# EDM-Research/Real-time-Neural-Rendering-of-LiDAR-Point-Clouds

Measured on AMD Instinct MI355X. Metric: Mpoints/sec projected + frames/sec at 1920x1080, higher is better.
Workload: dtype f32

## Files before the change

real-time-neural-rendering-of-lidar-point-clouds_amd/csrc/rtr_kernels.h:

```cpp
#pragma once
#include <hip/hip_runtime.h>
#include <stdint.h>

#include "rtr_chunk_box.h"

namespace rtr {

struct Proj {
    float m[12];
};

constexpr uint32_t kPackMaxBits = 25;
struct PackedXyz {
    const uint4 *hdr;
    const uint32_t *planes;
    const uint32_t *planes_b;
};
constexpr uint64_t pack_b_dwords(uint64_t units) { return (units * 2 + 256 + 16 + 15) & ~15ull; }
constexpr uint64_t pack_total_dwords(uint64_t units) { return pack_b_dwords(units) + units * 6 + 16; }

struct Cloud {
    const float *x, *y, *z;
    const uint32_t *rgba;
    uint64_t n;
    int grid;
    int incoherent;
    PackedXyz pk;
    const float *spread;
    float absmax[3];
    Clip clip;
    Keep keep;
};

struct FilterLevels {
    float *lv[9];
    int w[9], h[9];
    int levels;
};

constexpr int kMaxPeers = 16;
struct PeerSet {
    void *p[kMaxPeers];
};
struct OwnedTab;
struct Sliced {
    PeerSet src;
    size_t chunk;
    const uint32_t *occ_all;
    int peers;
    uint32_t *out;
    int rank;
    const OwnedTab *tab;
};
struct OwnedTab {
    const uint32_t *meta[kMaxPeers];
    const uint64_t *ext0[kMaxPeers];
    const uint64_t *dyn[kMaxPeers];
    const uint32_t *depth[kMaxPeers];
    const uint8_t *ximg[kMaxPeers];
};
struct TilePyr {
    FilterLevels L;
    uint32_t n_eff_rows;
    uint32_t *part_min, *part_max;
    int enable;
};
constexpr int kS0Shift = 12;
constexpr uint32_t kS0 = 1u << kS0Shift;
constexpr int kDirK = 21;
constexpr int kHeavyExtra = 512;
struct TileStore {
    uint64_t *ext0;
    uint32_t *meta;
    uint32_t seq;
    int nst, ntiles;
    int fill_shift;
};
constexpr int kFillShiftMax = 6;
struct StoreConsts {
    uint32_t *depth, *acc, *occ;
    uint64_t *dyn;
    uint64_t dyn_cap;
    uint32_t heavy, slice;
    uint32_t *err_host;
    uint32_t *split_host;
    uint32_t *entries_host;
};
__host__ __device__ constexpr size_t ts_align4(size_t x) { return (x + 3) & ~(size_t)3; }
__host__ __device__ constexpr size_t ts_off_count(int nst, int nt) { return ts_align4((size_t)nst << kFillShiftMax); }
__host__ __device__ constexpr size_t ts_off_tile_cnt(int nst, int nt) { return ts_off_count(nst, nt) + ts_align4((size_t)nst); }
__host__ __device__ constexpr size_t ts_off_hctr(int nst, int nt) { return ts_off_tile_cnt(nst, nt) + ts_align4((size_t)nt); }
__host__ __device__ constexpr size_t ts_off_items(int nst, int nt) { return ts_off_hctr(nst, nt) + ts_align4((size_t)nt); }
__host__ __device__ constexpr size_t ts_off_hdr(int nst, int nt) { return ts_off_items(nst, nt) + ((size_t)2 * nt + kHeavyExtra + 1) * 8; }
__host__ __device__ constexpr size_t ts_off_ticket(int nst, int nt) { return ts_off_hdr(nst, nt) + 32; }
__host__ __device__ constexpr size_t ts_off_pool(int nst, int nt) { return ts_off_ticket(nst, nt) + 2; }
__host__ __device__ constexpr size_t ts_off_dir(int nst, int nt) { return ts_off_pool(nst, nt) + 2; }
__host__ __device__ constexpr size_t ts_off_perm(int nst, int nt) { return ts_off_dir(nst, nt) + (size_t)nst * kDirK * 2; }
__host__ __device__ constexpr size_t ts_off_dbg(int nst, int nt) { return ts_off_perm(nst, nt) + ts_align4((size_t)nt); }
__host__ __device__ constexpr size_t ts_off_cnt4(int nst, int nt) { return ts_align4(ts_off_dbg(nst, nt) + 128); }
constexpr int kSubTickets = 32;
__host__ __device__ constexpr size_t ts_off_sub(int nst, int nt) { return ts_off_cnt4(nst, nt) + (size_t)nt * 4; }
__host__ __device__ constexpr size_t ts_off_order(int nst, int nt) { return ts_off_sub(nst, nt) + (size_t)kSubTickets * 32; }
// ... 204 lines not shown
```

real-time-neural-rendering-of-lidar-point-clouds_amd/csrc/rtr_kernels.hip:

```cpp
#include "rtr_device.h"
#include "rtr_lane_test.h"
#include "rtr_remove_index.h"
#include "rtr_extract_index.h"

#include <hip/hip_ext.h>
#include <hip/hip_fp16.h>

#include <type_traits>

namespace rtr {

__global__ __launch_bounds__(kBlock) void k_clear(uint4 *__restrict__ depth4, uint4 *__restrict__ acc4,
                                                  size_t n_depth4, size_t n_acc4, uint32_t *depth, size_t npix) {
    size_t i = (size_t)blockIdx.x * kBlock + threadIdx.x;
    size_t stride = (size_t)gridDim.x * kBlock;
    const uint4 e = make_uint4(RTR_EMPTY, RTR_EMPTY, RTR_EMPTY, RTR_EMPTY);
    const uint4 z = make_uint4(0, 0, 0, 0);
    for (size_t j = i; j < n_acc4; j += stride) acc4[j] = z;
    for (size_t j = i; j < n_depth4; j += stride) depth4[j] = e;
    for (size_t j = n_depth4 * 4 + i; j < npix; j += stride) depth[j] = RTR_EMPTY;
}

void launch_clear(hipStream_t s, uint32_t *depth, uint32_t *acc, size_t npix) {
    size_t n_acc4 = npix, n_depth4 = npix / 4;
// ... 263 lines not shown
                 project_point(P, X1.z, Y1.z, Z1.z, W, H, fW, fH, d) ^ project_point(P, X1.w, Y1.w, Z1.w, W, H, fW, fH, d);
        }
        if (i < n4) {
            Quad q = project_quad(x4, y4, z4, i, P, W, H, fW, fH);
            h += (uint32_t)(q.pix[0] ^ q.pix[1] ^ q.pix[2] ^ q.pix[3]);
        }
    } else {
        for (uint64_t i = (uint64_t)blockIdx.x * kBlock + threadIdx.x; i < n4; i += stride) {
            if (V == 0) {
                Quad q = project_quad(x4, y4, z4, i, P, W, H, fW, fH);
                h += (uint32_t)(q.pix[0] ^ q.pix[1] ^ q.pix[2] ^ q.pix[3]);
            } else if (V == 3) {
                float4 X = x4[i], Y = y4[i], Z = z4[i];
                float d;
                h += project_point(P, X.x, Y.x, Z.x, W, H, fW, fH, d) ^ project_point(P, X.y, Y.y, Z.y, W, H, fW, fH, d) ^
                     project_point(P, X.z, Y.z, Z.z, W, H, fW, fH, d) ^ project_point(P, X.w, Y.w, Z.w, W, H, fW, fH, d);
            } else if (V == 4) {
                float4 X = ld_stream(x4 + i), Y = ld_stream(y4 + i), Z = ld_stream(z4 + i);
                h += __float_as_uint(X.x) ^ __float_as_uint(Y.y) ^ __float_as_uint(Z.z) ^ __float_as_uint(X.w) ^
                     __float_as_uint(Y.x) ^ __float_as_uint(Z.y);
            } else {
                float4 X = ld_stream(x4 + i), Y = ld_stream(y4 + i), Z = ld_stream(z4 + i);
                const float xs[4] = {X.x, X.y, X.z, X.w}, ys[4] = {Y.x, Y.y, Y.z, Y.w}, zs[4] = {Z.x, Z.y, Z.z, Z.w};
#pragma unroll
                for (int k = 0; k < 4; ++k) {
                    float rx = f_add(fmaf(P.m[2], zs[k], fmaf(P.m[1], ys[k], f_mul(P.m[0], xs[k]))), P.m[3]);
                    float ry = f_add(fmaf(P.m[6], zs[k], fmaf(P.m[5], ys[k], f_mul(P.m[4], xs[k]))), P.m[7]);
                    float rz = f_add(fmaf(P.m[10], zs[k], fmaf(P.m[9], ys[k], f_mul(P.m[8], xs[k]))), P.m[11]);
                    float inv = __builtin_amdgcn_rcpf(rz);
                    float fu = rintf(f_mul(rx, inv)), fv = rintf(f_mul(ry, inv));
                    bool ok = (rz > 0.0f) && (fu >= 0.0f) && (fu < fW) && (fv >= 0.0f) && (fv < fH);
                    h += ok ? (uint32_t)((int)fv * W + (int)fu) : 0xFFFFFFFFu;
                }
            }
        }
    }
    if (h == 0x12345678u) sink[0] = h;
}

void launch_stream_probe(hipStream_t s, const Cloud &c, const Proj &P, int W, int H, uint32_t *sink, int variant) {
    uint64_t n4 = (c.n + 3) / 4;
    if (n4 == 0) return;
    dim3 g(point_grid(n4, c.grid)), b(kBlock);
    const float4 *x = (const float4 *)c.x, *y = (const float4 *)c.y, *z = (const float4 *)c.z;
    switch (variant) {
        case 1: hipLaunchKernelGGL(k_stream_probe<1>, g, b, 0, s, x, y, z, n4, P, W, H, sink); break;
        case 2: hipLaunchKernelGGL(k_stream_probe<2>, g, b, 0, s, x, y, z, n4, P, W, H, sink); break;
        case 3: hipLaunchKernelGGL(k_stream_probe<3>, g, b, 0, s, x, y, z, n4, P, W, H, sink); break;
        case 4: hipLaunchKernelGGL(k_stream_probe<4>, g, b, 0, s, x, y, z, n4, P, W, H, sink); break;
        default: hipLaunchKernelGGL(k_stream_probe<0>, g, b, 0, s, x, y, z, n4, P, W, H, sink); break;
    }
}

constexpr int kTileH = 32;
#ifndef RTR_TILE_THREADS
#define RTR_TILE_THREADS 512
#define RTR_TILE_BATCH 8
#define RTR_TILE_WAVES 6
#endif
constexpr int kTileThreads = RTR_TILE_THREADS;
#ifndef RTR_TILE0_THREADS
#define RTR_TILE0_THREADS 256
#endif
constexpr int kTileThreadsCompact = RTR_TILE0_THREADS;
#ifndef RTR_TILE0_WAVES
#define RTR_TILE0_WAVES 8
#define RTR_TILE0_SWEEP 4
#endif
#ifndef RTR_TILE0_HEAD
#define RTR_TILE0_HEAD 1
#endif
#ifndef RTR_TILE0_AHEAD
#define RTR_TILE0_AHEAD 1
#endif
#ifndef RTR_TILE0_BATCH
#define RTR_TILE0_BATCH 8
#endif
constexpr int kTileBatch = RTR_TILE_BATCH;
#ifndef RTR_T1_RING
#define RTR_T1_RING 3
#endif
#ifndef RTR_T1_LEAD
#define RTR_T1_LEAD 4
#endif
#ifndef RTR_T1_WAVES
#define RTR_T1_WAVES 5
#endif
constexpr int kSplitGrid = 256;
constexpr int kPer2 = kTileBatch / 2, kPer4 = kTileBatch / 4;
constexpr int kMaxGroups = RTR_MAX_GROUPS;
constexpr int kMaxSegs = 4 * kDirK;
#ifdef RTR_EXPERIMENT
#define RTR_XP(bit) ((xp & (bit)) != 0)
#define RTR_STAMP(S, slot) do { if (threadIdx.x == 0) ts_dbg(S)[slot] = wall_clock64(); } while (0)
#else
#define RTR_XP(bit) false
#define RTR_STAMP(S, slot) do { } while (0)
#endif

struct TileGeom {
    int tw_shift;
    int tiles_x, tiles_y, ntiles;
    int stx, sty, nst;
};

__host__ __device__ inline TileGeom tile_geom(int W, int H) {
    TileGeom g;
    g.tw_shift = 5;
    g.tiles_x = (W + 31) >> 5;
    g.tiles_y = (H + kTileH - 1) / kTileH;
    if (g.tiles_x * g.tiles_y > 4096) {
        g.tw_shift = 6;
        g.tiles_x = (W + 63) >> 6;
    }
    g.ntiles = g.tiles_x * g.tiles_y;
    g.stx = (W + 31) >> 5;
    g.sty = (H + 15) >> 4;
    g.nst = g.stx * g.sty;
    return g;
}

int tile_count(int W, int H) { return tile_geom(W, H).ntiles; }
int storage_tile_count(int W, int H) { return tile_geom(W, H).nst; }

__device__ __forceinline__ unsigned long long make_entry(uint32_t depth_bits, uint32_t pix9, uint32_t colour) {
    return ((unsigned long long)depth_bits << 33) | ((unsigned long long)pix9 << 24) | (unsigned long long)(colour & 0xFFFFFFu);
}

__device__ __forceinline__ void store_error(const TileStore &S, uint32_t code) { atomicOr(ts_hdr(S) + kHdrErrLive, code); }
__device__ __forceinline__ void store_error_now(const TileStore &S, uint32_t code) {
    store_error(S, code);
    typedef uint32_t __attribute__((address_space(1))) *gu32_t;
    uint32_t *const host = ts_consts(S)->err_host;
    if (host) *(volatile gu32_t)host = code;
}

__device__ __forceinline__ unsigned long long extent_alloc(const TileStore &S, uint32_t st, uint32_t v) {
    const int k = 32 - __clz((int)(v >> kS0Shift));
    const uint32_t start = kS0 << (k - 1);
    if (v != start) return 0ull;
    const unsigned long long base = atomicAdd(ts_pool(S), (unsigned long long)start);
    const unsigned long long e = (base << 24) | (unsigned long long)S.seq;
    __hip_atomic_store(ts_dir(S) + (size_t)st * kDirK + k, e, __ATOMIC_RELAXED, __HIP_MEMORY_SCOPE_AGENT);
    return e;
}
__device__ __forceinline__ uint64_t *extent_slot(const TileStore &S, uint32_t st, uint32_t v, unsigned long long own) {
    const int k = 32 - __clz((int)(v >> kS0Shift));
    const uint32_t start = kS0 << (k - 1);
    unsigned long long e = own;
    if (e == 0ull) {
        const unsigned long long *d = ts_dir(S) + (size_t)st * kDirK + k;
        int polls = 0;
        for (;;) {
            e = __hip_atomic_load(d, __ATOMIC_RELAXED, __HIP_MEMORY_SCOPE_AGENT);
            if ((uint32_t)(e & 0xFFFFFFull) == S.seq) break;
            if (++polls > (1 << 22)) {
                store_error(S, 1u);
                return nullptr;
            }
            __builtin_amdgcn_s_sleep(4);
        }
    }
    const unsigned long long base = e >> 24;
    const StoreConsts *sc = ts_consts(S);
    if (base + start > sc->dyn_cap) {
        store_error(S, 2u);
// ... 266 lines not shown
    if (threadIdx.x == 0) {
        sum = mx = over = 0;
        for (int k = 0; k < nw; ++k) {
            sum += s_w[k];
            mx = s_w[8 + k] > mx ? s_w[8 + k] : mx;
            over += s_w[16 + k];
        }
        uint32_t *const hdr = ts_hdr(S);
        hdr[kHdrItems] = (uint32_t)S.ntiles;
        hdr[kHdrSplitItems] = 0u;
        hdr[kHdrEntries] = sum;
        hdr[kHdrHeaviest] = mx;
        hdr[kHdrSlice] = sc->slice < 1u ? 1u : sc->slice;
        hdr[kHdrSplitTiles] = 0u;
        typedef uint32_t __attribute__((address_space(1))) *gu32_t;
        if (sc->split_host) *(volatile gu32_t)sc->split_host = over ? 1u : 0u;
        if (sc->entries_host) *(volatile gu32_t)sc->entries_host = sum;
        *flag = 0u;
    }
}
__device__ void lean_frame_end(const TileStore &S, int parity) {
    uint32_t *const hdr = ts_hdr(S);
    const int t = threadIdx.x;
    if (t < 64) {
        unsigned long long cc = 0ull;
        if (t < kSubTickets) {
            cc = *ts_sub_colour(S, (uint32_t)t);
            *ts_sub_colour(S, (uint32_t)t) = 0ull;
        }
        uint32_t c32 = (uint32_t)cc;
#pragma unroll
        for (int off = 32; off > 0; off >>= 1) c32 += __shfl_xor(c32, off, 64);
        if (t == 0) {
            hdr[kHdrColourChunks] = c32;
            const StoreConsts *const sc = ts_consts(S);
            const uint32_t err = __hip_atomic_load(hdr + kHdrErrLive, __ATOMIC_RELAXED, __HIP_MEMORY_SCOPE_AGENT);
            hdr[kHdrError] = err;
            if (err) {
                typedef uint32_t __attribute__((address_space(1))) *gu32_t;
                hdr[kHdrErrLive] = 0u;
                if (sc->err_host) *(volatile gu32_t)sc->err_host = err;
            }
            *ts_pool(S) = 0ull;
            ts_lflag(S)[parity] = 1u;
        }
    }
    __shared__ uint32_t s_fold[24];
    lean_fold(S, parity ^ 1, s_fold);
    __syncthreads();
    next_frame_order(S, parity, true);
}
__global__ __launch_bounds__(kBlock) void k_lean_fold(TileStore S, int parity) {
    __shared__ uint32_t s_fold[24];
    lean_fold(S, parity, s_fold);
}
void launch_lean_fold(hipStream_t s, int W, int H, const TileStore &S, int parity) {
    (void)W, (void)H;
    hipLaunchKernelGGL(k_lean_fold, dim3(1), dim3(kBlock), 0, s, S, parity);
}


struct ViewTab {
    Proj P[kMaxViews];
    LaneTest lt[kMaxViews];
    TileStore S[kMaxViews];
    const float *spread;
    int count;
};

template <bool CULL, bool GROUPS, bool PACKED, bool CTEST, bool MV, class... Filter>
__global__ __launch_bounds__(kBlock, (PACKED && !CULL && !MV) ? RTR_T1_WAVES : 4) void k_project_bin(const float4 *__restrict__ x4, const float4 *__restrict__ y4,
                                                        const float4 *__restrict__ z4,
                                                        const uint4 *__restrict__ rgba4, uint32_t n4, Proj P, int W,
                                                        int H, TileStore S, const float *__restrict__ bounds,
                                                        int clear_split, uint32_t cblock, int xp, LaneTest lt, Filter... filter) {
    constexpr bool CLIP = sizeof...(Filter) > 0, KEEP = sizeof...(Filter) > 1;
    const Clip no_clip{};
    const Keep no_keep{};
    const Clip &clip = filter_clip(no_clip, filter...);
    const Keep &kmask = filter_keep(no_keep, filter...);
    (void)xp;
    const ViewTab *const vt = MV ? reinterpret_cast<const ViewTab *>(bounds) : nullptr;
    const float *const spread = CULL ? nullptr : (MV ? vt->spread : bounds);
    const bool lane_test = (clear_split & 4) == 0;
    const uint4 *const pk_hdr = reinterpret_cast<const uint4 *>(x4);
    const uint32_t *const pk_planes = reinterpret_cast<const uint32_t *>(y4);
    const uint32_t *const pk_planes_b = reinterpret_cast<const uint32_t *>(z4);
    const float fW = (float)W, fH = (float)H;
    const float hiW = f_add(fW, 0.25f), hiH = f_add(fH, 0.25f);
    const int lane = threadIdx.x & 63;
    const uint32_t stx = (uint32_t)(W + 31) >> 5;
    uint32_t *fill = ts_fill(S);
    const uint32_t nchunks = (n4 + 63u) / 64u, NW = gridDim.x * (kBlock / 64), wave = blockIdx.x * (kBlock / 64) + (threadIdx.x >> 6);
    const uint32_t R = (nchunks + NW - 1u) / NW;
#ifdef RTR_EXPERIMENT
    const unsigned long long t_wave0 = wall_clock64();
    if (lane == 0 && (wave & 63u) == 0u) atomicMax(ts_dbg(S) + 59, ~t_wave0);
#endif
    const uint32_t auto_groups = ts_hdr(S)[kHdrEntries] > n4 ? 16u : ((PACKED && !CULL && GROUPS && R >= 16u) ? 5u : 1u);
    const uint32_t G = cblock < 1u ? auto_groups : (cblock > gridDim.x ? gridDim.x : cblock);
    const uint32_t phase = (uint32_t)((uint64_t)((blockIdx.x * G) / gridDim.x) * R / G);
    auto chunk_of = [&](uint32_t q) -> uint32_t {
        uint32_t r = q + phase;
        r = r >= R ? r - R : r;
        const uint32_t c = r * NW + wave;
        return (q < R && c < nchunks) ? c : nchunks;
    };
    struct Rows { float4 X, Y, Z; float rz[4]; };
    float mv[12];
#pragma unroll
    for (int k = 0; k < 12; ++k) {
        mv[k] = P.m[k];
        asm volatile("" : "+v"(mv[k]));
    }
    float nzfront = -lt.zfront;
    if constexpr (!PACKED) asm volatile("" : "+v"(nzfront));
    auto use_view = [&](uint32_t v) {
        if constexpr (MV) {
            S = vt->S[v];
            fill = ts_fill(S);
#pragma unroll
            for (int k = 0; k < 12; ++k) {
                mv[k] = vt->P[v].m[k];
                asm volatile("" : "+v"(mv[k]));
            }
            lt = vt->lt[v];
            nzfront = -lt.zfront;
            if constexpr (!PACKED) asm volatile("" : "+v"(nzfront));
        } else {
            (void)v;
        }
    };
#define RTR_M(k) mv[k]
    auto project_rows = [&](const float4 &X, const float4 &Y, const float4 &Z, Rows &r) {
        const float xs[4] = {X.x, X.y, X.z, X.w}, ys[4] = {Y.x, Y.y, Y.z, Y.w}, zs[4] = {Z.x, Z.y, Z.z, Z.w};
        r.X = X, r.Y = Y, r.Z = Z;
#pragma unroll
        for (int k = 0; k < 4; ++k) r.rz[k] = f_add(fmaf(RTR_M(10), zs[k], fmaf(RTR_M(9), ys[k], f_mul(RTR_M(8), xs[k]))), RTR_M(11));
    };
    auto lane_maybe = [&](float x0, float y0, float z0, float sp, bool live) -> bool {
        const float rz0 = f_add(fmaf(RTR_M(10), z0, fmaf(RTR_M(9), y0, f_mul(RTR_M(8), x0))), RTR_M(11));
        const float sz = f_mul(sp, lt.lz);
        const bool front = live && (f_add(rz0, sz) > nzfront);
        if (__ballot(front) == 0ull) return false;
        const float rx0 = f_add(fmaf(RTR_M(2), z0, fmaf(RTR_M(1), y0, f_mul(RTR_M(0), x0))), RTR_M(3));
        const float ry0 = f_add(fmaf(RTR_M(6), z0, fmaf(RTR_M(5), y0, f_mul(RTR_M(4), x0))), RTR_M(7));
        const float m = fminf(fminf(fmaf(hiW, rz0, -rx0), fmaf(hiH, rz0, -ry0)), fminf(fmaf(0.75f, rz0, rx0), fmaf(0.75f, rz0, ry0)));
        const bool out = (int)(f_sub(rz0, sz) > lt.zsafe) & (int)(m < -f_mul(sp, lt.lall));
        return __ballot(front && !out) != 0ull;
    };
    uint32_t n_colour = 0;
    uint32_t kst = kKeepAll;
    (void)kst;
    auto do_quad = [&](uint32_t i, bool live, const Rows &r) {
        const float *rz = r.rz;
        const bool front = live && (fmaxf(fmaxf(rz[0], rz[1]), fmaxf(rz[2], rz[3])) > 0.0f);
        if (__ballot(front) == 0ull) return;
        float rx[4], ry[4];
        {
            const float xs[4] = {r.X.x, r.X.y, r.X.z, r.X.w}, ys[4] = {r.Y.x, r.Y.y, r.Y.z, r.Y.w}, zs[4] = {r.Z.x, r.Z.y, r.Z.z, r.Z.w};
#pragma unroll
            for (int k = 0; k < 4; ++k) {
                rx[k] = f_add(fmaf(RTR_M(2), zs[k], fmaf(RTR_M(1), ys[k], f_mul(RTR_M(0), xs[k]))), RTR_M(3));
                ry[k] = f_add(fmaf(RTR_M(6), zs[k], fmaf(RTR_M(5), ys[k], f_mul(RTR_M(4), xs[k]))), RTR_M(7));
            }
        }
        bool maybe[4], any = false;
#pragma unroll
        for (int k = 0; k < 4; ++k) {
            const float z = rz[k];
            const float m = fminf(fminf(fmaf(hiW, z, -rx[k]), fmaf(hiH, z, -ry[k])), fminf(fmaf(0.75f, z, rx[k]), fmaf(0.75f, z, ry[k])));
            const bool out = (z > 1e-30f) && (m < 0.0f);
            maybe[k] = live && (z > 0.0f) && !out;
            any = any || maybe[k];
        }
        if (__ballot(any) == 0ull || RTR_XP(64)) return;
        if constexpr (CLIP) {
            const float xs[4] = {r.X.x, r.X.y, r.X.z, r.X.w}, ys[4] = {r.Y.x, r.Y.y, r.Y.z, r.Y.w}, zs[4] = {r.Z.x, r.Z.y, r.Z.z, r.Z.w};
            any = false;
#pragma unroll
            for (int k = 0; k < 4; ++k) {
                maybe[k] = maybe[k] && clip_keep(clip, xs[k], ys[k], zs[k]);
                any = any || maybe[k];
            }
            if (__ballot(any) == 0ull) return;
        }
        if constexpr (KEEP) {
            if (kst != kKeepAll) {
                const uint32_t c = (uint32_t)__builtin_amdgcn_readfirstlane((int)(i >> 6));
                const uint32_t kb = keep_bits(kmask, c, (uint32_t)lane);
                any = false;
#pragma unroll
                for (int k = 0; k < 4; ++k) {
                    maybe[k] = maybe[k] && ((kb >> k) & 1u);
                    any = any || maybe[k];
                }
                if (__ballot(any) == 0ull) return;
            }
        }
        bool in[4];
        uint32_t st[4], pix[4];
        unsigned long long pm[4];
#pragma unroll
        for (int k = 0; k < 4; ++k) {
            in[k] = false;
            st[k] = 0;
            pix[k] = 0;
            pm[k] = 0ull;
            if (__ballot(maybe[k]) == 0ull) continue;
            float inv = 1.0f / rz[k];
            float fu = rintf(f_mul(rx[k], inv));
            float fv = rintf(f_mul(ry[k], inv));
            in[k] = maybe[k] && (fu >= 0.0f) && (fu < fW) && (fv >= 0.0f) && (fv < fH);
            pm[k] = __ballot(in[k]);
            if (in[k]) {
                const int u = (int)fu, v = (int)fv;
                st[k] = (uint32_t)(v >> 4) * stx + (uint32_t)(u >> 5);
                pix[k] = (uint32_t)(((v & 15) << 5) | (u & 31));
            }
        }
        if ((pm[0] | pm[1] | pm[2] | pm[3]) == 0ull || RTR_XP(8)) return;
        n_colour += 1u;
        const uint4 col = rgba4[i];
        int grp[4] = {-1, -1, -1, -1};
        uint32_t rank[4] = {0, 0, 0, 0};
        uint32_t covered = 0;
#pragma clang diagnostic push
#pragma clang diagnostic ignored "-Wuninitialized"
#pragma clang diagnostic ignored "-Wsometimes-uninitialized"
        uint32_t claim[kMaxGroups];
#pragma clang diagnostic pop
        int ng = 0;
#pragma unroll
        for (int it = 0; it < (GROUPS ? kMaxGroups : 0); ++it) {
            const int kk = pm[0] ? 0 : (pm[1] ? 1 : (pm[2] ? 2 : (pm[3] ? 3 : -1)));
            if (kk < 0) continue;
            const unsigned long long pk = kk == 0 ? pm[0] : (kk == 1 ? pm[1] : (kk == 2 ? pm[2] : pm[3]));
            const uint32_t sk = kk == 0 ? st[0] : (kk == 1 ? st[1] : (kk == 2 ? st[2] : st[3]));
            const int first = __ffsll((long long)pk) - 1;
            const uint32_t lead = (uint32_t)__builtin_amdgcn_readlane((int)sk, first);
            uint32_t total = 0, lower = 0;
            bool gk[4];
#pragma unroll
            for (int k = 0; k < 4; ++k) {
                const unsigned long long m = __ballot(st[k] == lead) & pm[k];
                gk[k] = __builtin_amdgcn_inverse_ballot_w64(m);
                lower += __builtin_amdgcn_mbcnt_hi((uint32_t)(m >> 32), __builtin_amdgcn_mbcnt_lo((uint32_t)m, 0u));
                total += (uint32_t)__popcll(m);
                pm[k] &= ~m;
            }
#pragma unroll
            for (int k = 0; k < 4; ++k)
                if (gk[k]) {
                    grp[k] = it;
                    rank[k] = lower++;
                }
            if (lane == it) claim[it] = atomicAdd(fill + ((size_t)lead << S.fill_shift), total);
            ng = it + 1;
            covered += total;
            if (it == 3 && covered <= 8u) {
                pm[0] = pm[1] = pm[2] = pm[3] = 0ull;
            }
        }
#pragma unroll
        for (int k = 0; k < 4; ++k)
            if (in[k] && grp[k] < 0) {
                rank[k] = atomicAdd(fill + ((size_t)st[k] << S.fill_shift), 1u);
                grp[k] = kMaxGroups;
            }
        uint32_t bsel[4] = {0u, 0u, 0u, 0u};
        auto select_base = [&](auto self, auto it_tag) -> void {
            constexpr int it = decltype(it_tag)::value;
            if constexpr (it < kMaxGroups) {
                if (it < ng) {
                    const uint32_t b_it = (uint32_t)__builtin_amdgcn_readlane((int)claim[it], it);
#pragma unroll
                    for (int k = 0; k < 4; ++k) bsel[k] = grp[k] == it ? b_it : bsel[k];
                    self(self, std::integral_constant<int, it + 1>{});
                }
            }
        };
        if (!RTR_XP(16)) select_base(select_base, std::integral_constant<int, 0>{});
        const uint32_t cs[4] = {col.x, col.y, col.z, col.w};
        uint32_t v[4];
        bool dyn = false;
#pragma unroll
        for (int k = 0; k < 4; ++k) {
            v[k] = bsel[k] + rank[k];
            dyn = dyn || (in[k] && v[k] >= kS0);
        }
        if (RTR_XP(4)) return;
        if (RTR_XP(512)) {
            if ((v[0] ^ v[1] ^ v[2] ^ v[3]) == 0x7FFFFFFFu) fill[0] = 0u;
            return;
        }
        if (__ballot(dyn) == 0ull) {
            const bool quad = in[0] && in[1] && in[2] && in[3] && grp[0] < kMaxGroups && grp[0] == grp[1] &&
                              grp[0] == grp[2] && grp[0] == grp[3];
            if (quad) {
                typedef unsigned long long ull2 __attribute__((ext_vector_type(2)));
                struct __attribute__((packed, aligned(8))) Pair { ull2 v; };
                Pair *dst = reinterpret_cast<Pair *>(S.ext0 + ((size_t)st[0] << kS0Shift) + v[0]);
                ull2 a, b;
                a.x = make_entry(__float_as_uint(rz[0]), pix[0], cs[0]);
                a.y = make_entry(__float_as_uint(rz[1]), pix[1], cs[1]);
                b.x = make_entry(__float_as_uint(rz[2]), pix[2], cs[2]);
                b.y = make_entry(__float_as_uint(rz[3]), pix[3], cs[3]);
                dst[0].v = a;
                dst[1].v = b;
            } else {
#pragma unroll
                for (int k = 0; k < 4; ++k)
                    if (in[k]) S.ext0[((size_t)st[k] << kS0Shift) + v[k]] = make_entry(__float_as_uint(rz[k]), pix[k], cs[k]);
            }
        } else {
            unsigned long long own[4];
#pragma unroll
            for (int k = 0; k < 4; ++k) own[k] = (in[k] && v[k] >= kS0) ? extent_alloc(S, st[k], v[k]) : 0ull;
            __builtin_amdgcn_wave_barrier();
#pragma unroll
            for (int k = 0; k < 4; ++k)
                if (in[k]) {
                    uint64_t *slot = v[k] < kS0 ? S.ext0 + ((size_t)st[k] << kS0Shift) + v[k] : extent_slot(S, st[k], v[k], own[k]);
                    typedef uint64_t __attribute__((address_space(1))) *gslot_t;
                    if (slot) *(gslot_t)slot = make_entry(__float_as_uint(rz[k]), pix[k], cs[k]);
                }
        }
    };

    if (!CULL && PACKED) {
        constexpr int kRing = RTR_T1_RING, kLead = RTR_T1_LEAD, kRingH = kRing + kLead;
        static_assert(((kRing + 1) & kRing) == 0 && ((kRingH + 1) & kRingH) == 0, "ring sizes: powers of two");
        typedef uint32_t __attribute__((address_space(3))) lds_u32;
        constexpr int kSlotDw = 256;
        __shared__ __attribute__((aligned(16))) uint32_t s_ring[kBlock / 64][kRing + 1][kSlotDw];
        __shared__ __attribute__((aligned(16))) uint32_t s_rhdr[kBlock / 64][kRingH + 1][8];
        const uint32_t ring_lds = (uint32_t)__builtin_amdgcn_readfirstlane((int)(uint32_t)(uintptr_t)(lds_u32 *)s_ring[threadIdx.x >> 6]);
        const uint32_t rhdr_lds = (uint32_t)__builtin_amdgcn_readfirstlane((int)(uint32_t)(uintptr_t)(lds_u32 *)s_rhdr[threadIdx.x >> 6]);
        const uint32_t lane16 = 16u * (uint32_t)lane;
        const uint32_t c_first = (uint32_t)__builtin_amdgcn_readfirstlane((int)(phase * NW + wave)), c_wrap = R * NW + wave;
        auto next_chunk = [&](uint32_t c) -> uint32_t {
            c += NW;
            return c >= c_wrap ? c - R * NW : c;
        };
        auto req_hdr = [&](uint32_t q, uint32_t c) {
            const uint32_t cc = c < nchunks ? c : nchunks - 1u;
            const uint32_t voff = 32u * cc + lane16, lds = rhdr_lds + 32u * (q & (uint32_t)kRingH);
            if (lane < 2) asm volatile("s_mov_b32 m0, %2\n\tglobal_load_lds_dwordx4 %0, %1" : : "v"(voff), "s"(pk_hdr), "s"(lds) : "memory", "m0");
        };
        auto req_data = [&](uint32_t q) {
            const lds_u32 *const hs = (const lds_u32 *)(uintptr_t)(rhdr_lds + 32u * (q & (uint32_t)kRingH));
            const uint32_t lo = (uint32_t)__builtin_amdgcn_readfirstlane((int)hs[4]), hi = (uint32_t)__builtin_amdgcn_readfirstlane((int)hs[5]);
            const uint8_t *src = reinterpret_cast<const uint8_t *>(pk_planes) + (((((uint64_t)hi) << 32) | (uint64_t)lo) << 3);
            const uint32_t lds = ring_lds + 4u * (uint32_t)kSlotDw * (q & (uint32_t)kRing);
            if (lane < 48) asm volatile("s_mov_b32 m0, %2\n\tglobal_load_lds_dwordx4 %0, %1" : : "v"(lane16), "s"(src), "s"(lds) : "memory", "m0");
        };
#ifdef RTR_EXPERIMENT
        uint32_t xp_sink = 0;
#endif
        typedef uint32_t u32x4_l __attribute__((ext_vector_type(4)));
        typedef u32x4_l __attribute__((address_space(3))) lds_u32x4;
        auto chunk_body = [&](const lds_u32 *slot, const u32x4_l &g0, const u32x4_l &g1, uint32_t c, uint32_t vmask) {
            if constexpr (KEEP && (MV || !CTEST)) {
                kst = keep_state(kmask, c);
                if (!CTEST && kst == kKeepNone) return;
            }
            const uint32_t ww = (uint32_t)__builtin_amdgcn_readfirstlane((int)g0.w);
            const uint32_t bx = g0.x, by = g0.y, bz = g0.z;
            const uint32_t wx = ww & 63u, wy = (ww >> 6) & 63u, wz = (ww >> 12) & 63u;
            ChunkRawA raw;
            uint32_t px, py, pz;
            asm("v_mul_u32_u24 %0, %1, %2" : "=v"(px) : "s"(wx), "v"(lane));
            asm("v_mul_u32_u24 %0, %1, %2" : "=v"(py) : "s"(wy), "v"(lane));
            asm("v_mul_u32_u24 %0, %1, %2" : "=v"(pz) : "s"(wz), "v"(lane));
            {
                const uint32_t ix = px >> 5, iy = 2u * wx + (py >> 5), iz = 2u * (wx + wy) + (pz >> 5);
                raw.a[0].d[0] = slot[ix], raw.a[0].d[1] = slot[ix + 1];
                raw.a[1].d[0] = slot[iy], raw.a[1].d[1] = slot[iy + 1];
                raw.a[2].d[0] = slot[iz], raw.a[2].d[1] = slot[iz + 1];
            }
            Rows r;
            float4 X, Y, Z;
#ifdef RTR_EXPERIMENT
            if (RTR_XP(128)) {
                xp_sink ^= raw.a[0].d[0] ^ raw.a[1].d[1] ^ raw.a[2].d[0] ^ raw.a[0].d[1] ^ raw.a[1].d[0] ^ raw.a[2].d[1];
                return;
            }
#endif
            bool cand = true;
            const uint32_t sp_c = (uint32_t)__builtin_amdgcn_readfirstlane((int)g1.z);
            if (lane_test && !(ww & kPackWideFlag) && sp_c < 0x7F000000u) {
                auto value0 = [&](uint32_t d0, uint32_t d1, uint32_t prod, uint32_t b, uint32_t base) -> float {
                    uint32_t x;
                    asm("v_and_or_b32 %0, %1, %2, %3" : "=v"(x) : "v"(__builtin_amdgcn_alignbit(d1, d0, prod)), "s"((1u << b) - 1u), "v"(base));
                    return __uint_as_float(x);
                };
                const float x0 = value0(raw.a[0].d[0], raw.a[0].d[1], px, wx, bx);
                const float y0 = value0(raw.a[1].d[0], raw.a[1].d[1], py, wy, by);
                const float z0 = value0(raw.a[2].d[0], raw.a[2].d[1], pz, wz, bz);
                if constexpr (MV) {
                    uint32_t kept = 0u;
                    for (uint32_t m = vmask; m; m &= m - 1u) {
                        const uint32_t v = (uint32_t)__builtin_ctz(m);
                        use_view(v);
                        if (lane_maybe(x0, y0, z0, __uint_as_float(sp_c), true)) kept |= 1u << v;
                    }
                    vmask = kept;
                    cand = kept != 0u;
                } else {
                    cand = lane_maybe(x0, y0, z0, __uint_as_float(sp_c), true);
                }
            }
            if (!cand) return;
            uint32_t i_c = c * 64u + (uint32_t)lane;
            const bool live_c = i_c < n4;
            i_c = live_c ? i_c : n4 - 1u;
            {
                const uint32_t sbx = (uint32_t)__builtin_amdgcn_readfirstlane((int)bx), sby = (uint32_t)__builtin_amdgcn_readfirstlane((int)by);
                const uint32_t sbz = (uint32_t)__builtin_amdgcn_readfirstlane((int)bz);
                const uint4 hc0 = make_uint4(sbx, sby, sbz, ww);
                const uint4 hc1 = make_uint4((uint32_t)__builtin_amdgcn_readfirstlane((int)g1.x), (uint32_t)__builtin_amdgcn_readfirstlane((int)g1.y), 0u, 0u);
                ChunkRaw raw_b;
#ifdef RTR_EXPERIMENT
                if (RTR_XP(1024)) {
#pragma unroll
                    for (int a = 0; a < 3; ++a) raw_b.a[a].d[0] = raw.a[a].d[0], raw_b.a[a].d[1] = raw.a[a].d[1], raw_b.a[a].d[2] = raw.a[a].d[0], raw_b.a[a].d[3] = raw.a[a].d[1];
                } else
#endif
                raw_b = load_chunk_b(pk_planes_b, hc0, hc1, lane);
                if constexpr (CTEST) {
#pragma unroll
                    for (int a = 0; a < 3; ++a) asm volatile("" : "+v"(raw_b.a[a].d[0]), "+v"(raw_b.a[a].d[1]), "+v"(raw_b.a[a].d[2]), "+v"(raw_b.a[a].d[3]));
                }
                unpack_chunk(raw, raw_b, ww, sbx, sby, sbz, X, Y, Z, lane);
                if constexpr (!MV) project_rows(X, Y, Z, r);
            }
            if constexpr (MV) {
                for (uint32_t m = vmask; m; m &= m - 1u) {
                    use_view((uint32_t)__builtin_ctz(m));
                    project_rows(X, Y, Z, r);
                    do_quad(i_c, live_c, r);
                }
                return;
            }
#ifdef RTR_EXPERIMENT
            if (RTR_XP(256)) {
                xp_sink ^= __float_as_uint(r.rz[0]) ^ __float_as_uint(r.rz[1]) ^ __float_as_uint(r.rz[2]) ^ __float_as_uint(r.rz[3]);
                return;
            }
#endif
            do_quad(i_c, live_c, r);
        };
        if constexpr (CTEST) {
            uint4 cur0, cur1;
            uint32_t ksum = 0u;
            uint32_t qb = 0;
            unsigned long long pmask = 0ull;
            auto load_batch = [&](uint32_t q0, uint4 &h0, uint4 &h1) {
                const uint32_t c = chunk_of(q0 + (uint32_t)lane);
                const uint32_t cc = c < nchunks ? c : nchunks - 1u;
                h0 = pk_hdr[2 * (size_t)cc];
                h1 = pk_hdr[2 * (size_t)cc + 1];
                if constexpr (KEEP) ksum = kmask.sum[cc];
            };
            auto test_batch = [&]() {
                const uint32_t c = chunk_of(qb + (uint32_t)lane);
                bool keep = c < nchunks;
                float lo[3], hi[3];
                uint32_t vm = MV ? (1u << vt->count) - 1u : 0u;
                const uint32_t wbox = cur1.w;
                if (MV && keep && chunk_box(cur0.x, cur0.y, cur0.z, cur0.w, wbox, lo, hi)) {
                    vm = 0u;
                    for (int v = 0; v < vt->count; ++v) {
                        float m[12];
#pragma unroll
                        for (int k = 0; k < 12; ++k) {
                            m[k] = vt->P[v].m[k];
                            asm volatile("" : "+v"(m[k]));
                        }
                        if (!box_outside(frustum_planes(m, fW, fH), lo, hi)) vm |= 1u << v;
                    }
                    if (CLIP && clip_box_outside(clip, lo, hi)) vm = 0u;
                    keep = vm != 0u;
                } else if (!MV && keep && chunk_box(cur0.x, cur0.y, cur0.z, cur0.w, wbox, lo, hi)) {
                    float m[12];
#pragma unroll
                    for (int k = 0; k < 12; ++k) {
                        m[k] = mv[k];
                        asm volatile("" : "+v"(m[k]));
                    }
                    keep = !box_outside(frustum_planes(m, fW, fH), lo, hi);
                    if (CLIP) keep = keep && !clip_box_outside(clip, lo, hi);
                }
                if constexpr (KEEP) keep = keep && ksum != kKeepNone;
                cur1.w = MV ? (c | vm << 24) : (KEEP ? (c | ksum << 30) : c);
                asm volatile("" : "+v"(cur0.x), "+v"(cur0.y), "+v"(cur0.z), "+v"(cur0.w), "+v"(cur1.x), "+v"(cur1.y), "+v"(cur1.z));
                pmask = __ballot(keep);
            };
            auto req = [&](uint32_t k) {
                while (pmask == 0ull && qb + 64u < R) {
                    qb += 64u;
                    load_batch(qb, cur0, cur1);
                    test_batch();
                }
                const uint32_t hs = rhdr_lds + 32u * (k & (uint32_t)kRing), lds = ring_lds + 4u * (uint32_t)kSlotDw * (k & (uint32_t)kRing);
                if (pmask != 0ull) {
                    const int l = __ffsll((long long)pmask) - 1;
                    pmask &= pmask - 1ull;
                    if (lane == l) {
                        *(lds_u32x4 *)(uintptr_t)hs = u32x4_l{cur0.x, cur0.y, cur0.z, cur0.w};
                        *(lds_u32x4 *)(uintptr_t)(hs + 16u) = u32x4_l{cur1.x, cur1.y, cur1.z, cur1.w};
                    }
                    const uint32_t lo = (uint32_t)__builtin_amdgcn_readlane((int)cur1.x, l), hi = (uint32_t)__builtin_amdgcn_readlane((int)cur1.y, l);
                    const uint8_t *src = reinterpret_cast<const uint8_t *>(pk_planes) + (((((uint64_t)hi) << 32) | (uint64_t)lo) << 3);
                    if (lane < 48) asm volatile("s_mov_b32 m0, %2\n\tglobal_load_lds_dwordx4 %0, %1" : : "v"(lane16), "s"(src), "s"(lds) : "memory", "m0");
                } else {
                    if (lane == 0) *(lds_u32 *)(uintptr_t)(hs + 28u) = ~0u;
                    if (lane < 48) asm volatile("s_mov_b32 m0, %2\n\tglobal_load_lds_dwordx4 %0, %1" : : "v"(lane16), "s"(pk_planes), "s"(lds) : "memory", "m0");
                }
            };
            load_batch(0u, cur0, cur1);
            test_batch();
#pragma unroll
            for (int k = 0; k < kRing; ++k) req((uint32_t)k);
            for (uint32_t k = 0;; ++k) {
                req(k + (uint32_t)kRing);
                asm volatile("s_waitcnt vmcnt(%0)" : : "n"(kRing) : "memory");
                const lds_u32 *const slot = (const lds_u32 *)(uintptr_t)(ring_lds + 4u * (uint32_t)kSlotDw * (k & (uint32_t)kRing));
                const lds_u32 *const hs = (const lds_u32 *)(uintptr_t)(rhdr_lds + 32u * (k & (uint32_t)kRing));
                const u32x4_l g0 = *reinterpret_cast<const lds_u32x4 *>(hs);
                const u32x4_l g1 = *reinterpret_cast<const lds_u32x4 *>(hs + 4);
                const uint32_t cw = (uint32_t)__builtin_amdgcn_readfirstlane((int)g1.w);
                if constexpr (KEEP && !MV) {
                    if ((cw & 0x3FFFFFFFu) >= nchunks) break;
                    kst = cw >> 30;
                    chunk_body(slot, g0, g1, cw & 0x3FFFFFFFu, 0u);
                    continue;
                }
                if (MV ? cw == ~0u : cw >= nchunks) break;
                chunk_body(slot, g0, g1, MV ? (cw & 0xFFFFFFu) : cw, cw >> 24);
            }
        } else {
            uint32_t c_req = c_first;
#pragma unroll
            for (int k = 0; k < kRingH; ++k) {
                req_hdr((uint32_t)k, (uint32_t)k < R ? c_req : nchunks);
                c_req = next_chunk(c_req);
            }
#pragma unroll
            for (int k = 0; k < kRing; ++k) {
                asm volatile("s_waitcnt vmcnt(%0)" : : "n"(kRingH - 1) : "memory");
                req_data((uint32_t)k);
            }
            asm volatile("s_waitcnt vmcnt(0)" ::: "memory");
            uint32_t c_use = c_first;
            for (uint32_t q = 0; q < R; ++q) {
                req_hdr(q + (uint32_t)kRingH, q + (uint32_t)kRingH < R ? c_req : nchunks);
                c_req = next_chunk(c_req);
                asm volatile("s_waitcnt vmcnt(%0)" : : "n"(2 * kLead) : "memory");
                req_data(q + (uint32_t)kRing);
                asm volatile("s_waitcnt vmcnt(%0)" : : "n"(2 * kRing) : "memory");
                const lds_u32 *const slot = (const lds_u32 *)(uintptr_t)(ring_lds + 4u * (uint32_t)kSlotDw * (q & (uint32_t)kRing));
                const lds_u32 *const hs = (const lds_u32 *)(uintptr_t)(rhdr_lds + 32u * (q & (uint32_t)kRingH));
                const u32x4_l g0 = *reinterpret_cast<const lds_u32x4 *>(hs);
                const u32x4_l g1 = *reinterpret_cast<const lds_u32x4 *>(hs + 4);
                const uint32_t c = c_use;
                c_use = next_chunk(c_use);
                if (c >= nchunks) continue;
                chunk_body(slot, g0, g1, c, 0u);
            }
        }
        asm volatile("s_waitcnt vmcnt(0)" ::: "memory");
#ifdef RTR_EXPERIMENT
        if (xp_sink == 0x12345678u) fill[0] = 0u;
#endif

    } else if (!CULL) {
        float4 X = make_float4(0.f, 0.f, 0.f, 0.f), Y = X, Z = X;
        uint32_t i = 0, spb = 0x7F800000u, kst_f = kKeepAll;
        bool have = false, live = false;
        auto fetch = [&](uint32_t q) {
            const uint32_t c = (uint32_t)__builtin_amdgcn_readfirstlane((int)(q < R ? chunk_of(q) : nchunks));
            have = c < nchunks;
            if constexpr (KEEP) {
                kst_f = have ? keep_state(kmask, c) : kKeepAll;
                if (kst_f == kKeepNone) have = false;
            }
            if (have) {
                i = c * 64u + (uint32_t)lane;
                live = i < n4;
                const uint32_t ic = live ? i : n4 - 1u;
                if (spread) spb = __float_as_uint(spread[c]);
                X = ld_stream(x4 + ic);
                Y = ld_stream(y4 + ic);
                Z = ld_stream(z4 + ic);
            }
        };
        fetch(0);
        if constexpr (MV) {
            for (uint32_t q = 0; q < R; ++q) {
                Rows r;
                const bool have_c = have, live_c = live;
                const uint32_t i_c = i < n4 ? i : n4 - 1u;
                const float4 Xc = X, Yc = Y, Zc = Z;
                const uint32_t spc = spb;
                if constexpr (KEEP) kst = kst_f;
                fetch(q + 1);
                if (!have_c) continue;
                for (int v = 0; v < vt->count; ++v) {
                    use_view((uint32_t)v);
// ... 2664 lines not shown
```

Before: 1.058 million.

## Stage packed B-plane data into the LDS ring with async global-to-LDS loads

```diff
diff --git a/real-time-neural-rendering-of-lidar-point-clouds_amd/csrc/rtr_b_ring.h b/real-time-neural-rendering-of-lidar-point-clouds_amd/csrc/rtr_b_ring.h
--- /dev/null
+++ b/real-time-neural-rendering-of-lidar-point-clouds_amd/csrc/rtr_b_ring.h
@@ -0,0 +1,38 @@
+#pragma once
+#include <stdint.h>
+
+#if defined(__HIPCC__)
+#define RTR_BR_HD __host__ __device__ inline
+#else
+#define RTR_BR_HD inline
+#endif
+
+namespace rtr {
+
+constexpr uint32_t kBRingADw = 256;
+constexpr uint32_t kBRingReqs = 3;
+constexpr uint32_t kBRingReqBytes = 1024;
+constexpr uint32_t kBRingMaxBytes = 24u * 96u;
+constexpr uint32_t kBRingOverRead = 16;
+constexpr uint32_t kBRingSlotDw = kBRingADw + (kBRingMaxBytes + kBRingOverRead) / 4;
+constexpr uint32_t kBRingSpareBytes = 16;
+static_assert(kBRingReqs * kBRingReqBytes >= kBRingMaxBytes && (kBRingReqs - 1) * kBRingReqBytes < kBRingMaxBytes, "requests per survivor");
+static_assert(kBRingSlotDw % 4 == 0, "slots start on 16-byte boundaries");
+
+RTR_BR_HD uint32_t b_ring_width(uint32_t widths, int axis) { return (widths >> (6 * axis)) & 63u; }
+RTR_BR_HD uint32_t b_ring_bytes(uint32_t widths) { return 24u * (b_ring_width(widths, 0) + b_ring_width(widths, 1) + b_ring_width(widths, 2)); }
+RTR_BR_HD uint32_t b_ring_bytes16(uint32_t widths) { return (b_ring_bytes(widths) + 15u) & ~15u; }
+RTR_BR_HD uint32_t b_ring_req_left(uint32_t nb16, uint32_t j) { return nb16 > kBRingReqBytes * j ? nb16 - kBRingReqBytes * j : 0u; }
+RTR_BR_HD bool b_ring_lane_active(uint32_t nb16, uint32_t j, uint32_t lane) {
+    const uint32_t left = b_ring_req_left(nb16, j);
+    return 16u * lane < (left > 16u ? left : 16u);
+}
+RTR_BR_HD uint32_t b_ring_lane_src(uint32_t nb16, uint32_t j, uint32_t lane) { return (b_ring_req_left(nb16, j) ? kBRingReqBytes * j : 0u) + 16u * lane; }
+RTR_BR_HD uint32_t b_ring_lane_dst(uint32_t j, uint32_t lane) { return 4u * kBRingADw + kBRingReqBytes * j + 16u * lane; }
+RTR_BR_HD uint32_t b_ring_axis_dw(uint32_t widths, int axis, uint32_t lane) {
+    uint32_t before = 0;
+    for (int a = 0; a < axis; ++a) before += b_ring_width(widths, a);
+    return kBRingADw + 6u * before + ((3u * b_ring_width(widths, axis) * lane) >> 5);
+}
+
+}
diff --git a/real-time-neural-rendering-of-lidar-point-clouds_amd/csrc/rtr_kernels.h b/real-time-neural-rendering-of-lidar-point-clouds_amd/csrc/rtr_kernels.h
--- a/real-time-neural-rendering-of-lidar-point-clouds_amd/csrc/rtr_kernels.h
+++ b/real-time-neural-rendering-of-lidar-point-clouds_amd/csrc/rtr_kernels.h
@@ -2,6 +2,7 @@
 #include <hip/hip_runtime.h>
 #include <stdint.h>
 
+#include "rtr_b_ring.h"
 #include "rtr_chunk_box.h"
 
 namespace rtr {
@@ -17,7 +18,9 @@
     const uint32_t *planes_b;
 };
 constexpr uint64_t pack_b_dwords(uint64_t units) { return (units * 2 + 256 + 16 + 15) & ~15ull; }
-constexpr uint64_t pack_total_dwords(uint64_t units) { return pack_b_dwords(units) + units * 6 + 16; }
+constexpr uint64_t kPackSpareDwB = 16;
+constexpr uint64_t pack_total_dwords(uint64_t units) { return pack_b_dwords(units) + units * 6 + kPackSpareDwB; }
+static_assert(kPackSpareDwB * 4 >= kBRingSpareBytes && kPackSpareDwB * 4 >= 16, "B spare: the last lane's over-read, the point kernel's ring requests (rtr_b_ring.h)");
 
 struct Cloud {
     const float *x, *y, *z;
diff --git a/real-time-neural-rendering-of-lidar-point-clouds_amd/csrc/rtr_kernels.hip b/real-time-neural-rendering-of-lidar-point-clouds_amd/csrc/rtr_kernels.hip
--- a/real-time-neural-rendering-of-lidar-point-clouds_amd/csrc/rtr_kernels.hip
+++ b/real-time-neural-rendering-of-lidar-point-clouds_amd/csrc/rtr_kernels.hip
@@ -369,6 +369,15 @@
 #endif
 #ifndef RTR_T1_LEAD
 #define RTR_T1_LEAD 4
+#endif
+#ifndef RTR_T1_BRING
+#define RTR_T1_BRING 1
+#endif
+#ifndef RTR_T1_BRING_LANE_TEST
+#define RTR_T1_BRING_LANE_TEST 0
+#endif
+#ifndef RTR_T1_BRING_AHEAD
+#define RTR_T1_BRING_AHEAD 1
 #endif
 #ifndef RTR_T1_WAVES
 #define RTR_T1_WAVES 5
@@ -801,12 +810,22 @@
     (void)xp;
     const ViewTab *const vt = MV ? reinterpret_cast<const ViewTab *>(bounds) : nullptr;
     const float *const spread = CULL ? nullptr : (MV ? vt->spread : bounds);
-    const bool lane_test = (clear_split & 4) == 0;
+    constexpr bool kBRingInst = PACKED && !CULL && CTEST && !MV && RTR_T1_BRING != 0;
+    const bool lane_test = (kBRingInst && RTR_T1_BRING_LANE_TEST == 0) ? false : (clear_split & 4) == 0;
     const uint4 *const pk_hdr = reinterpret_cast<const uint4 *>(x4);
     const uint32_t *const pk_planes = reinterpret_cast<const uint32_t *>(y4);
     const uint32_t *const pk_planes_b = reinterpret_cast<const uint32_t *>(z4);
     const float fW = (float)W, fH = (float)H;
     const float hiW = f_add(fW, 0.25f), hiH = f_add(fH, 0.25f);
+    auto hi_bounds = [&](float &hw, float &hh) {
+        if constexpr (kBRingInst) {
+            int w = W, h = H;
+            asm volatile("" : "+s"(w), "+s"(h));
+            hw = f_add((float)w, 0.25f), hh = f_add((float)h, 0.25f);
+        } else {
+            hw = hiW, hh = hiH;
+        }
+    };
     const int lane = threadIdx.x & 63;
     const uint32_t stx = (uint32_t)(W + 31) >> 5;
     uint32_t *fill = ts_fill(S);
@@ -864,7 +883,9 @@
         if (__ballot(front) == 0ull) return false;
         const float rx0 = f_add(fmaf(RTR_M(2), z0, fmaf(RTR_M(1), y0, f_mul(RTR_M(0), x0))), RTR_M(3));
         const float ry0 = f_add(fmaf(RTR_M(6), z0, fmaf(RTR_M(5), y0, f_mul(RTR_M(4), x0))), RTR_M(7));
-        const float m = fminf(fminf(fmaf(hiW, rz0, -rx0), fmaf(hiH, rz0, -ry0)), fminf(fmaf(0.75f, rz0, rx0), fmaf(0.75f, rz0, ry0)));
+        float hw, hh;
+        hi_bounds(hw, hh);
+        const float m = fminf(fminf(fmaf(hw, rz0, -rx0), fmaf(hh, rz0, -ry0)), fminf(fmaf(0.75f, rz0, rx0), fmaf(0.75f, rz0, ry0)));
         const bool out = (int)(f_sub(rz0, sz) > lt.zsafe) & (int)(m < -f_mul(sp, lt.lall));
         return __ballot(front && !out) != 0ull;
     };
@@ -885,10 +906,12 @@
             }
         }
         bool maybe[4], any = false;
+        float hw, hh;
+        hi_bounds(hw, hh);
 #pragma unroll
         for (int k = 0; k < 4; ++k) {
             const float z = rz[k];
-            const float m = fminf(fminf(fmaf(hiW, z, -rx[k]), fmaf(hiH, z, -ry[k])), fminf(fmaf(0.75f, z, rx[k]), fmaf(0.75f, z, ry[k])));
+            const float m = fminf(fminf(fmaf(hw, z, -rx[k]), fmaf(hh, z, -ry[k])), fminf(fmaf(0.75f, z, rx[k]), fmaf(0.75f, z, ry[k])));
             const bool out = (z > 1e-30f) && (m < 0.0f);
             maybe[k] = live && (z > 0.0f) && !out;
             any = any || maybe[k];
@@ -1048,10 +1071,14 @@
     };
 
     if (!CULL && PACKED) {
-        constexpr int kRing = RTR_T1_RING, kLead = RTR_T1_LEAD, kRingH = kRing + kLead;
+        constexpr bool BRING = kBRingInst;
+        constexpr int kLead = RTR_T1_LEAD;
+        constexpr int kRing = BRING ? RTR_T1_BRING_AHEAD : RTR_T1_RING, kRingH = BRING ? kRing : kRing + kLead;
+        constexpr int kReq = BRING ? 1 + (int)kBRingReqs : 1;
         static_assert(((kRing + 1) & kRing) == 0 && ((kRingH + 1) & kRingH) == 0, "ring sizes: powers of two");
         typedef uint32_t __attribute__((address_space(3))) lds_u32;
-        constexpr int kSlotDw = 256;
+        constexpr int kSlotDw = BRING ? (int)kBRingSlotDw : 256;
+        static_assert(!BRING || (kBlock / 64) * (kRing + 1) * (kSlotDw * 4 + 32) <= 31818, "LDS budget of the B ring");
         __shared__ __attribute__((aligned(16))) uint32_t s_ring[kBlock / 64][kRing + 1][kSlotDw];
         __shared__ __attribute__((aligned(16))) uint32_t s_rhdr[kBlock / 64][kRingH + 1][8];
         const uint32_t ring_lds = (uint32_t)__builtin_amdgcn_readfirstlane((int)(uint32_t)(uintptr_t)(lds_u32 *)s_ring[threadIdx.x >> 6]);
@@ -1146,6 +1173,13 @@
                     for (int a = 0; a < 3; ++a) raw_b.a[a].d[0] = raw.a[a].d[0], raw_b.a[a].d[1] = raw.a[a].d[1], raw_b.a[a].d[2] = raw.a[a].d[0], raw_b.a[a].d[3] = raw.a[a].d[1];
                 } else
 #endif
+                if constexpr (BRING) {
+                    (void)hc1;
+                    const lds_u32 *const sb = slot + kBRingADw;
+                    const uint32_t jx = (3u * px) >> 5, jy = 6u * wx + ((3u * py) >> 5), jz = 6u * (wx + wy) + ((3u * pz) >> 5);
+#pragma unroll
+                    for (int d = 0; d < 4; ++d) raw_b.a[0].d[d] = sb[jx + d], raw_b.a[1].d[d] = sb[jy + d], raw_b.a[2].d[d] = sb[jz + d];
+                } else
                 raw_b = load_chunk_b(pk_planes_b, hc0, hc1, lane);
                 if constexpr (CTEST) {
 #pragma unroll
@@ -1223,6 +1257,33 @@
                     test_batch();
                 }
                 const uint32_t hs = rhdr_lds + 32u * (k & (uint32_t)kRing), lds = ring_lds + 4u * (uint32_t)kSlotDw * (k & (uint32_t)kRing);
+                if constexpr (BRING) {
+                    auto issue = [&](const uint8_t *src, const uint8_t *src_b, uint32_t nb16) {
+                        if (lane < 48) asm volatile("s_mov_b32 m0, %2\n\tglobal_load_lds_dwordx4 %0, %1" : : "v"(lane16), "s"(src), "s"(lds) : "memory", "m0");
+#pragma unroll
+                        for (uint32_t j = 0; j < kBRingReqs; ++j) {
+                            const uint32_t left = b_ring_req_left(nb16, j);
+                            const uint32_t voff = (left ? kBRingReqBytes * j : 0u) + lane16, ldb = lds + 4u * kBRingADw + kBRingReqBytes * j;
+                            if (lane16 < (left > 16u ? left : 16u))
+                                asm volatile("s_mov_b32 m0, %2\n\tglobal_load_lds_dwordx4 %0, %1" : : "v"(voff), "s"(src_b), "s"(ldb) : "memory", "m0");
+                        }
+                    };
+                    if (pmask != 0ull) {
+                        const int l = __ffsll((long long)pmask) - 1;
+                        pmask &= pmask - 1ull;
+                        if (lane == l) {
+                            *(lds_u32x4 *)(uintptr_t)hs = u32x4_l{cur0.x, cur0.y, cur0.z, cur0.w};
+                            *(lds_u32x4 *)(uintptr_t)(hs + 16u) = u32x4_l{cur1.x, cur1.y, cur1.z, cur1.w};
+                        }
+                        const uint32_t lo = (uint32_t)__builtin_amdgcn_readlane((int)cur1.x, l), hi = (uint32_t)__builtin_amdgcn_readlane((int)cur1.y, l);
+                        const uint64_t unit = (((uint64_t)hi) << 32) | (uint64_t)lo;
+                        issue(reinterpret_cast<const uint8_t *>(pk_planes) + (unit << 3), reinterpret_cast<const uint8_t *>(pk_planes_b) + unit * 24u,
+                              b_ring_bytes16((uint32_t)__builtin_amdgcn_readlane((int)cur0.w, l)));
+                    } else {
+                        if (lane == 0) *(lds_u32 *)(uintptr_t)(hs + 28u) = ~0u;
+                        issue(reinterpret_cast<const uint8_t *>(pk_planes), reinterpret_cast<const uint8_t *>(pk_planes_b), 0u);
+                    }
+                } else
                 if (pmask != 0ull) {
                     const int l = __ffsll((long long)pmask) - 1;
                     pmask &= pmask - 1ull;
@@ -1244,7 +1305,7 @@
             for (int k = 0; k < kRing; ++k) req((uint32_t)k);
             for (uint32_t k = 0;; ++k) {
                 req(k + (uint32_t)kRing);
-                asm volatile("s_waitcnt vmcnt(%0)" : : "n"(kRing) : "memory");
+                asm volatile("s_waitcnt vmcnt(%0)" : : "n"(kReq * kRing) : "memory");
                 const lds_u32 *const slot = (const lds_u32 *)(uintptr_t)(ring_lds + 4u * (uint32_t)kSlotDw * (k & (uint32_t)kRing));
                 const lds_u32 *const hs = (const lds_u32 *)(uintptr_t)(rhdr_lds + 32u * (k & (uint32_t)kRing));
                 const u32x4_l g0 = *reinterpret_cast<const lds_u32x4 *>(hs);
```

After: 1.076 million (median of 6 runs). Within noise of the previous version (+1.7%).
